# xjtu-omics/SVision

Measured on AMD Instinct MI355X. Metric: candidate SV sites/sec (encode+CNN), higher is better.
Workload: dtype f32

## Files before the change

### include/svx_experimental.h

```cpp
#ifndef SVX_EXPERIMENTAL_H
#define SVX_EXPERIMENTAL_H
#include "svx.h"
#ifdef __cplusplus
extern "C" {
#endif

size_t svx_cigar_scan_flat_ws_bytes(uint64_t n_words_max);
int svx_cigar_scan_flat(const uint32_t* d_cigar, const uint64_t* d_cig_off, const int32_t* d_ref_start, uint32_t n_aln,
                        uint64_t n_words_max, int32_t min_sv, SvxGap* d_gaps, uint64_t gaps_cap, uint32_t* d_gap_off,
                        int32_t* d_stats, void* d_ws, uint64_t ws_bytes, void* stream);

int            svx_bgzf_inflate(const uint8_t* d_comp, const uint64_t* d_src_off, const uint32_t* d_src_len,
                                const uint64_t* d_dst_off, uint32_t n_blocks, uint8_t* d_out, uint32_t* d_status, void* stream);
int            svx_bgzf_inflate_lds(const uint8_t* d_comp, const uint64_t* d_src_off, const uint32_t* d_src_len,
                                    const uint64_t* d_dst_off, uint32_t n_blocks, uint8_t* d_out, uint32_t* d_status, void* stream);
int            svx_bgzf_inflate_private(const uint8_t* d_comp, const uint64_t* d_src_off, const uint32_t* d_src_len,
                                        const uint64_t* d_dst_off, uint32_t n_blocks, uint8_t* d_out, uint32_t* d_status, void* stream);
int            svx_bgzf_inflate_wave(const uint8_t* d_comp, const uint64_t* d_src_off, const uint32_t* d_src_len,
                                     const uint64_t* d_dst_off, uint32_t n_blocks, uint8_t* d_out, uint32_t* d_status, void* stream);

int            svx_bgzf_inflate_fast_lz(const uint8_t* d_comp, const uint64_t* d_src_off, const uint32_t* d_src_len,
                                        const uint64_t* d_dst_off, uint32_t n_blocks, uint64_t inflated_bytes, uint8_t* d_out,
                                        uint32_t* d_status, void* d_ws, uint64_t ws_bytes, int lz_kernel, void* stream_tokens,
                                        void* stream_lz);

#ifdef __cplusplus
}
#endif
#endif
```

### svision_amd/_lib.py

```python
import ctypes
import os

_HERE = os.path.dirname(os.path.abspath(__file__))
LIB_PATH = os.path.join(_HERE, "libsvx.so")

SVX_OK = 0
SVX_EINVAL = -1
SVX_ECAPACITY = -2
SVX_ELAUNCH = -3
LAYOUT_NHWC = 0
LAYOUT_NCHW = 1
IMG = 227
GAP_INS = 1
GAP_DEL = 2

_vp, _u32, _i32, _u64, _sz = ctypes.c_void_p, ctypes.c_uint32, ctypes.c_int32, ctypes.c_uint64, ctypes.c_size_t
SYMBOLS = {
    "svx_version": (ctypes.c_int, []),
    "svx_strerror": (ctypes.c_char_p, [ctypes.c_int]),
    "svx_crc32c": (_u32, [_vp, _sz]),
    "svx_cigar_scan_ws_bytes": (_sz, [_u32, _u64]),
    "svx_cigar_scan": (ctypes.c_int, [_vp, _vp, _vp, _u32, _u64, _i32, _vp, _u64, _vp, _vp, _vp, _u64, _u32, _vp]),
    "svx_rasterize": (ctypes.c_int, [_vp, _u32, _vp, ctypes.c_int, ctypes.POINTER(ctypes.c_float), _vp]),
    "svx_encode_conv1": (ctypes.c_int, [_vp, _u32, _vp, _vp, _vp, ctypes.c_int, _u32, ctypes.c_float, ctypes.c_float,
# ... 54 lines not shown
    "svx_record_retag_measure": (ctypes.c_int, [_vp, _vp, _u32, _vp, _vp, _i32, _vp, _vp, _vp]),
    "svx_record_retag_write": (ctypes.c_int, [_vp, _vp, _u32, _vp, _vp, _i32, _vp, _vp, _vp, _vp]),
    "svx_record_tags_measure": (ctypes.c_int, [_vp, _vp, _u32, _vp, _vp, _vp, _vp]),
    "svx_record_tags_write": (ctypes.c_int, [_vp, _vp, _u32, _vp, _vp, _vp, _vp, _vp]),
    "svx_bgzf_deflate": (ctypes.c_int, [_vp, _vp, _u32, _vp, _vp, _vp, _vp]),
    "svx_bgzf_deflate_dyn_ws_bytes": (_sz, [_u32]),
    "svx_bgzf_deflate_dyn": (ctypes.c_int, [_vp, _vp, _u32, _vp, _vp, _vp, _vp, _u64, _vp]),
    "svx_bgzf_pack": (ctypes.c_int, [_vp, _vp, _u32, _vp, _vp, _u64, _vp]),
    "svx_sam_lines_ws_bytes": (_sz, [_u64]),
    "svx_sam_lines": (ctypes.c_int, [_vp, _u64, _vp, _u64, _vp, _vp, _u64, _vp]),
    "svx_sam_measure": (ctypes.c_int, [_vp, _vp, _u32] + [_vp] * 4 + [_u32] + [_vp] * 5 + [_vp]),
    "svx_sam_encode": (ctypes.c_int, [_vp, _vp, _u32] + [_vp] * 4 + [_u32, _vp, _vp, ctypes.c_int64, _vp, _vp, _vp]),
    "svx_sam_pack_count": (ctypes.c_int, [_vp, _vp, _u32] + [_vp] * 4 + [_u32, ctypes.c_int] + [_vp] * 3 + [_vp]),
    "svx_sam_pack_extract": (ctypes.c_int, [_vp, _vp, _u32] + [_vp] * 4 + [_u32] + [_vp] * 12 + [_vp]),
    "svx_read_range": (ctypes.c_int, [ctypes.c_char_p, _u64, _u64, _vp, ctypes.c_int]),
    "svx_bgzf_index": (ctypes.c_int64, [_vp, _u64, _u64, _u64, _vp, _vp, _vp, _vp, _vp]),
    "svx_name_ids": (ctypes.c_int64, [_vp, _vp, _u64, _vp, _vp, _vp]),
    "svx_stage_open": (_vp, [ctypes.c_char_p, ctypes.c_int, _vp, ctypes.c_int, _vp, ctypes.c_int, _u64, ctypes.c_int, _vp]),
    "svx_stage_group": (ctypes.c_int64, [_vp, _vp, _u64, _vp, _vp, _vp, _u64]),
    "svx_stage_tables": (ctypes.c_int, [_vp, _vp, _vp, _vp, _vp, _u64]),
    "svx_stage_close": (None, [_vp]),
    "svx_bam_stream_open": (_vp, [ctypes.c_char_p, ctypes.c_int, ctypes.c_int, _vp, ctypes.c_int]),
    "svx_bam_stream_next": (_vp, [_vp, _vp]),
    "svx_bam_stream_close": (None, [_vp]),
}
EXPERIMENTAL = {
    "svx_cigar_scan_flat_ws_bytes": (_sz, [_u64]),
    "svx_cigar_scan_flat": (ctypes.c_int, [_vp, _vp, _vp, _u32, _u64, _i32, _vp, _u64, _vp, _vp, _vp, _u64, _vp]),
    "svx_bgzf_inflate": (ctypes.c_int, [_vp, _vp, _vp, _vp, _u32, _vp, _vp, _vp]),
    "svx_bgzf_inflate_wave": (ctypes.c_int, [_vp, _vp, _vp, _vp, _u32, _vp, _vp, _vp]),
    "svx_bgzf_inflate_lds": (ctypes.c_int, [_vp, _vp, _vp, _vp, _u32, _vp, _vp, _vp]),
    "svx_bgzf_inflate_private": (ctypes.c_int, [_vp, _vp, _vp, _vp, _u32, _vp, _vp, _vp]),
    "svx_bgzf_inflate_fast_lz": (ctypes.c_int, [_vp, _vp, _vp, _vp, _u32, _u64, _vp, _vp, _vp, _u64, ctypes.c_int, _vp, _vp]),
}


class SvxError(RuntimeError):
    pass


class SvxMissing(SvxError):
    """libsvx.so has not been built (as opposed to: built, but wrong)."""


_lib = None


ABI_VERSION = 420


def load():
    global _lib
    if _lib is None:
        if not os.path.exists(LIB_PATH):
            raise SvxMissing(
                f"{LIB_PATH} is missing: build it with `python -c 'import __graft_entry__ as g; g.build()'` "
                "or `make -C svision_amd/csrc` (hipcc --offload-arch=gfx950). There is no CPU fallback.")
        lib = ctypes.CDLL(LIB_PATH)
        for name, (res, args) in list(SYMBOLS.items()) + list(EXPERIMENTAL.items()):
            fn = getattr(lib, name)
            fn.restype = res
            fn.argtypes = args
        if lib.svx_version() != ABI_VERSION:
            raise SvxError(f"{LIB_PATH} reports ABI {lib.svx_version()}, this package binds {ABI_VERSION}: rebuild it (make -C svision_amd/csrc)")
        _lib = lib
    return _lib
# ... 7 lines not shown
```

### svision_amd/csrc/svx_dedup.hip

```cpp
#include "svx_raster_common.hpp"

namespace {

constexpr int KEY_BLOCK = 256, COMPACT_BLOCK = 1024, WAVE = 64;

__device__ inline bool key_eq(const uint4& a, const uint4& b) { return a.x == b.x && a.y == b.y && a.z == b.z && a.w == b.w; }

__global__ __launch_bounds__(KEY_BLOCK)
void first_kernel(const int32_t* __restrict__ records, uint32_t n, uint32_t* __restrict__ first, uint4* __restrict__ keys)
{
    __shared__ uint4 tile[KEY_BLOCK];
    const uint32_t i = blockIdx.x * KEY_BLOCK + threadIdx.x;
    const uint4 mine = i < n ? svx_raster::image_key(records + (size_t)i * 12) : uint4{0, 0, 0, 0};
    if (keys && i < n) keys[i] = mine;
    uint32_t f = i;
    for (uint32_t t = 0; t <= blockIdx.x; ++t) {
        const uint32_t j0 = t * KEY_BLOCK;
        __syncthreads();
        if (t == blockIdx.x) tile[threadIdx.x] = mine;
        else tile[threadIdx.x] = svx_raster::image_key(records + (size_t)(j0 + threadIdx.x) * 12);
        __syncthreads();
        if (f == i) {
            const uint32_t hi = min((uint32_t)KEY_BLOCK, i - j0);
            for (uint32_t j = 0; j < hi; ++j)
                if (key_eq(tile[j], mine)) { f = j0 + j; break; }
        }
    }
    if (i < n) first[i] = f;
}

__global__ __launch_bounds__(COMPACT_BLOCK)
void compact_kernel(const int32_t* __restrict__ records, uint32_t n, uint32_t* __restrict__ inv, uint32_t* __restrict__ row,
                    int32_t* __restrict__ unique, uint32_t* __restrict__ live)
{
    __shared__ uint32_t wave_sum[COMPACT_BLOCK / WAVE];
    __shared__ uint32_t s_base;
    const int t = threadIdx.x, lane = t & (WAVE - 1), wv = t / WAVE;
    const uint32_t block = blockDim.x;
    if (t == 0) s_base = 0;
    __syncthreads();
    for (uint32_t c0 = 0; c0 < n; c0 += block) {
        const uint32_t i = c0 + t;
        const bool is_first = i < n && inv[i] == i;
        const unsigned long long ball = __ballot(is_first);
        const uint32_t below = __popcll(ball & ((1ull << lane) - 1ull));
        if (lane == 0) wave_sum[wv] = __popcll(ball);
        __syncthreads();
        uint32_t before = s_base;
        for (int w = 0; w < wv; ++w) before += wave_sum[w];
        if (is_first) {
            const uint32_t c = before + below;
            row[i] = c;
#pragma unroll
            for (int e = 0; e < 12; ++e) unique[(size_t)c * 12 + e] = records[(size_t)i * 12 + e];
        }
        __syncthreads();
        if (t == 0) { uint32_t s = s_base; for (uint32_t w = 0; w < block / WAVE; ++w) s += wave_sum[w]; s_base = s; }
        __syncthreads();
    }
    const uint32_t n_live = s_base;
    for (uint32_t e = n_live * 12 + t; e < n * 12; e += block) unique[e] = records[e % 12];
    for (uint32_t i = t; i < n; i += block) inv[i] = row[inv[i]];
    if (t == 0) *live = n_live;
}

__global__ __launch_bounds__(COMPACT_BLOCK)
void dedup_small_kernel(const int32_t* __restrict__ records, uint32_t n, uint32_t* __restrict__ inv, int32_t* __restrict__ unique,
                        uint32_t* __restrict__ live, uint4* __restrict__ keys)
{
    constexpr uint32_t SCAN = 8;
    __shared__ uint4 tile[COMPACT_BLOCK];
    __shared__ uint32_t row[COMPACT_BLOCK];
    __shared__ uint32_t wave_sum[COMPACT_BLOCK / WAVE];
    const uint32_t i = threadIdx.x, lane = i & (WAVE - 1), wv = i / WAVE, block = blockDim.x;
    const uint4 mine = i < n ? svx_raster::image_key(records + (size_t)i * 12) : uint4{0, 0, 0, 0};
    if (keys && i < n) keys[i] = mine;
    tile[i] = mine;
    __syncthreads();
    uint32_t f = i;
    if (i < n)
        for (uint32_t j0 = 0; j0 < i && f == i; j0 += SCAN) {
            uint32_t hit = 0;
#pragma unroll
            for (uint32_t u = 0; u < SCAN; ++u)
                if (key_eq(tile[j0 + u], mine) && j0 + u < i) hit |= 1u << u;
            if (hit) f = j0 + __ffs(hit) - 1;
        }
    const bool is_first = i < n && f == i;
    const unsigned long long ball = __ballot(is_first);
    const uint32_t below = __popcll(ball & ((1ull << lane) - 1ull));
    if (lane == 0) wave_sum[wv] = __popcll(ball);
    __syncthreads();
    uint32_t before = 0, n_live = 0;
    for (uint32_t w = 0; w < block / WAVE; ++w) { if (w == wv) before = n_live; n_live += wave_sum[w]; }
    if (is_first) {
        const uint32_t c = before + below;
        row[i] = c;
#pragma unroll
        for (int e = 0; e < 12; ++e) unique[(size_t)c * 12 + e] = records[(size_t)i * 12 + e];
    }
    __syncthreads();
    if (i < n) inv[i] = row[f];
    for (uint32_t e = n_live * 12 + i; e < n * 12; e += block) unique[e] = records[e % 12];
    if (i == 0) *live = n_live;
}

__global__ __launch_bounds__(256)
void gather_rows_kernel(const float* __restrict__ src, const uint32_t* __restrict__ inv, float* __restrict__ dst, uint32_t n, uint32_t width)
{
    const uint32_t e = blockIdx.x * 256 + threadIdx.x;
    if (e >= n * width) return;
    const uint32_t i = e / width, c = e - i * width;
    dst[e] = src[(size_t)inv[i] * width + c];
}

}

extern "C" int svx_image_dedup(const int32_t* d_records, uint32_t n, int32_t* d_unique, uint32_t* d_inv, uint32_t* d_live,
                               uint32_t* d_keys, uint32_t* d_ws, void* stream)
{
    if (!d_live) return SVX_EINVAL;
    hipStream_t st = static_cast<hipStream_t>(stream);
    if (n == 0) return hipMemsetAsync(d_live, 0, sizeof(uint32_t), st) == hipSuccess ? SVX_OK : SVX_ELAUNCH;
    if (!d_records || !d_unique || !d_inv || !d_ws || n > (1u << 26)) return SVX_EINVAL;
    if (reinterpret_cast<uintptr_t>(d_keys) & 15u) return SVX_EINVAL;
    const uint32_t block = n >= COMPACT_BLOCK ? COMPACT_BLOCK : (n + WAVE - 1) / WAVE * WAVE;
    if (n <= COMPACT_BLOCK) {
        hipLaunchKernelGGL(dedup_small_kernel, dim3(1), dim3(block), 0, st, d_records, n, d_inv, d_unique, d_live, reinterpret_cast<uint4*>(d_keys));
        return hipGetLastError() == hipSuccess ? SVX_OK : SVX_ELAUNCH;
    }
    hipLaunchKernelGGL(first_kernel, dim3((n + KEY_BLOCK - 1) / KEY_BLOCK), dim3(KEY_BLOCK), 0, st, d_records, n, d_inv,
                       reinterpret_cast<uint4*>(d_keys));
    hipLaunchKernelGGL(compact_kernel, dim3(1), dim3(block), 0, st, d_records, n, d_inv, d_ws, d_unique, d_live);
    return hipGetLastError() == hipSuccess ? SVX_OK : SVX_ELAUNCH;
}

extern "C" int svx_gather_rows(const float* d_src, const uint32_t* d_inv, float* d_dst, uint32_t n, uint32_t width, void* stream)
{
    if (n == 0 || width == 0) return SVX_OK;
    if (!d_src || !d_inv || !d_dst || (uint64_t)n * width > 0xffffffffull) return SVX_EINVAL;
    const uint32_t total = n * width;
    hipLaunchKernelGGL(gather_rows_kernel, dim3((total + 255) / 256), dim3(256), 0, static_cast<hipStream_t>(stream), d_src, d_inv, d_dst, n, width);
    return hipGetLastError() == hipSuccess ? SVX_OK : SVX_ELAUNCH;
}
```

### svision_amd/csrc/svx_inflate2.hip

```cpp
#include <hip/hip_runtime.h>
#include <stdint.h>
#include <stdlib.h>
#include "../../include/svx.h"
#include "svx_lz_core.hpp"
#include "svx_lz_table_core.hpp"
#include "svx_wave_scan.hpp"

#ifndef SVX_TOK_DBG
#define SVX_TOK_DBG 0
#endif

namespace {

constexpr int LANES = 64;
#ifndef SVX_TOK_LB
#define SVX_TOK_LB 9
#define SVX_TOK_DB 7
#endif
#ifndef SVX_TOK_WAVES
#define SVX_TOK_WAVES 4
#endif
constexpr int LB = SVX_TOK_LB, DB = SVX_TOK_DB;
constexpr int LIT_CAP = (1 << LB) + (LB >= 9 ? 340 : 512), DIST_CAP = (1 << DB) + 528;
#ifndef SVX_TOK_SEG
#define SVX_TOK_SEG 512
#endif
constexpr int SEG_BITS = SVX_TOK_SEG;
constexpr int CHUNK_WORDS = LANES * SEG_BITS / 32 + 8;
enum { K_BAD = 0, K_LIT = 1, K_LEN = 2, K_EOB = 3, K_SUB = 4 };
enum { INF_OK = 0, INF_BAD_TYPE = 1, INF_BAD_STORED = 2, INF_BAD_TABLE = 3, INF_BAD_CODE = 4, INF_OUT_OVERRUN = 5, INF_IN_OVERRUN = 6, INF_SHORT = 7,
       INF_BAD_DIST = 8, INF_TOKENS_OVERFLOW = 10 };

__constant__ uint16_t LEN_BASE[29] = {3, 4, 5, 6, 7, 8, 9, 10, 11, 13, 15, 17, 19, 23, 27, 31, 35, 43, 51, 59, 67, 83, 99, 115, 131, 163, 195, 227, 258};
__constant__ uint8_t LEN_EXTRA[29] = {0, 0, 0, 0, 0, 0, 0, 0, 1, 1, 1, 1, 2, 2, 2, 2, 3, 3, 3, 3, 4, 4, 4, 4, 5, 5, 5, 5, 0};
__constant__ uint16_t DIST_BASE[30] = {1, 2, 3, 4, 5, 7, 9, 13, 17, 25, 33, 49, 65, 97, 129, 193, 257, 385, 513, 769, 1025, 1537, 2049, 3073, 4097, 6145, 8193, 12289, 16385, 24577};
__constant__ uint8_t DIST_EXTRA[30] = {0, 0, 0, 0, 1, 1, 2, 2, 3, 3, 4, 4, 5, 5, 6, 6, 7, 7, 8, 8, 9, 9, 10, 10, 11, 11, 12, 12, 13, 13};
__constant__ uint8_t CLEN_ORDER[19] = {16, 17, 18, 0, 8, 7, 9, 6, 10, 5, 11, 4, 12, 3, 13, 2, 14, 1, 15};

struct LitPayload {
    __device__ __forceinline__ uint32_t operator()(int s) const
    {
        if (s < 256) return (uint32_t)K_LIT << 4 | (uint32_t)s << 8;
        if (s == 256) return (uint32_t)K_EOB << 4;
        if (s - 257 >= 29) return (uint32_t)K_BAD << 4;
        return (uint32_t)K_LEN << 4 | (uint32_t)LEN_BASE[s - 257] << 8 | (uint32_t)LEN_EXTRA[s - 257] << 17;
    }
};
struct DistPayload {
    __device__ __forceinline__ uint32_t operator()(int s) const
    {
        return s >= 30 ? (uint32_t)K_BAD << 4 : ((uint32_t)K_LEN << 4 | (uint32_t)DIST_BASE[s] << 8 | (uint32_t)DIST_EXTRA[s] << 23);
    }
};
struct ClenPayload { __device__ __forceinline__ uint32_t operator()(int s) const { return (uint32_t)K_LIT << 4 | (uint32_t)s << 8; } };

struct Lds {
    uint32_t lit[LIT_CAP];
    uint32_t dist[DIST_CAP];
    uint32_t chunk[CHUNK_WORDS];
    __device__ __forceinline__ uint8_t* lens() { return reinterpret_cast<uint8_t*>(chunk) + 1024; }
    __device__ __forceinline__ uint8_t* cl() { return reinterpret_cast<uint8_t*>(chunk) + 1344; }
    __device__ __forceinline__ uint16_t* code() { return reinterpret_cast<uint16_t*>(chunk) + 704; }
};
static_assert(sizeof(Lds) <= 10240 && LANES * SEG_BITS / 8 >= 2048, "sixteen waves per CU; the builder's scratch fits the chunk buffer");

__device__ __forceinline__ int uni(int v) { return __builtin_amdgcn_readfirstlane(v); }
__device__ __forceinline__ void lds_fence() { __builtin_amdgcn_s_waitcnt(0xc07f); __builtin_amdgcn_wave_barrier(); }

struct HeadReader {
    const uint32_t* words;
    uint32_t cur, nxt;
    uint64_t chunk_next, word_end;
    int k;
    uint64_t buf;
    int cnt;
    uint32_t fed;
    __device__ __forceinline__ uint32_t fetch(uint64_t first) { const uint64_t i = first + threadIdx.x; return i < word_end ? words[i] : 0u; }
    __device__ __forceinline__ void refill()
    {
        if (cnt <= 32) {
            const uint32_t v = (uint32_t)__builtin_amdgcn_readlane((int)cur, k);
            if (++k == 64) { cur = nxt; nxt = fetch(chunk_next); chunk_next += 64; k = 0; }
            buf |= (uint64_t)v << cnt;
            cnt += 32;
        }
    }
    __device__ __forceinline__ void seek(const uint8_t* base, uint32_t bytes, uint32_t bit)
    {
        const uintptr_t a = reinterpret_cast<uintptr_t>(base) + (bit >> 3);
        words = reinterpret_cast<const uint32_t*>(a & ~(uintptr_t)3);
        word_end = ((reinterpret_cast<uintptr_t>(base) + bytes + 3) >> 2) - (reinterpret_cast<uintptr_t>(words) >> 2) + 1;
        cur = fetch(0); nxt = fetch(64); chunk_next = 128;
        k = 0; buf = 0; cnt = 0;
        refill();
        const int skip = (int)(a & 3) * 8 + (int)(bit & 7);
        buf >>= skip; cnt -= skip;
        fed = 0;
    }
    __device__ __forceinline__ uint32_t bits(int n)
    {
        refill();
        const uint32_t v = (uint32_t)buf & ((1u << n) - 1u);
        buf >>= n; cnt -= n; fed += (uint32_t)n;
        return v;
    }
};

template <class Payload>
__device__ int build_tables(const uint8_t* lens, int n, int root, uint32_t* tab, int cap, uint16_t* code_of, uint8_t* tmp, Payload payload)
{
    const int lane = threadIdx.x;
    const unsigned long long lt = (1ull << lane) - 1ull;
    int count[16];
#pragma unroll
    for (int l = 0; l < 16; ++l) count[l] = 0;
    for (int s0 = 0; s0 < n; s0 += LANES) {
        const int l = s0 + lane < n ? (int)lens[s0 + lane] : 0;
#pragma unroll
        for (int q = 1; q < 16; ++q) count[q] += (int)__popcll(__ballot(l == q));
    }
    int next[16], left = 1, code = 0;
    next[0] = 0;
#pragma unroll
    for (int l = 1; l <= 15; ++l) {
        left = (left << 1) - count[l];
        code = (code + (l > 1 ? count[l - 1] : 0)) << 1;
        next[l] = code;
    }
    if (left < 0) return 0;
    for (int s0 = 0; s0 < n; s0 += LANES) {
        const int l = s0 + lane < n ? (int)lens[s0 + lane] : 0;
        int mine = 0;
#pragma unroll
        for (int q = 1; q < 16; ++q) {
            const unsigned long long m = __ballot(l == q);
            if (l == q) mine = next[q] + (int)__popcll(m & lt);
            next[q] += (int)__popcll(m);
        }
        if (s0 + lane < n) code_of[s0 + lane] = (uint16_t)mine;
    }
    const int nroot = 1 << root;
    for (int i = lane; i < nroot; i += LANES) { tab[i] = 0; tmp[i] = 0; }
    lds_fence();
    for (int s0 = 0; s0 < n; s0 += LANES) {
// ... 73 lines not shown
    Tok k{(e >> 4) & 15u, used, (e >> 8) & 255u, 0u, 0u};
    if (k.kind != K_LEN) return k;
    const uint32_t xb = (e >> 17) & 7u;
    k.len = ((e >> 8) & 511u) + ((b.lo >> used) & ((1u << xb) - 1u));
    used += xb;
    const uint32_t db32 = __builtin_amdgcn_alignbit(b.hi, b.lo, used);
    uint32_t d = t.dist[db32 & ((1u << DB) - 1u)];
    uint32_t dused;
    if (((d >> 4) & 15u) == K_SUB) {
        d = t.dist[((d >> 8) & 0xfffu) + ((db32 >> DB) & ((1u << ((d >> 20) & 15u)) - 1u))];
        dused = DB + (d & 15u);
    } else dused = d & 15u;
    if (((d >> 4) & 15u) != K_LEN) { k.kind = K_BAD; k.used = used + dused; return k; }
    const uint32_t nb = (d >> 23) & 15u;
    k.dist = ((d >> 8) & 0x7fffu) + ((db32 >> dused) & ((1u << nb) - 1u));
    k.used = used + dused + nb;
    return k;
}

using svx_wave::wave_incl_scan;

__device__ __forceinline__ uint32_t wave_excl_sum(uint32_t v, uint32_t* total)
{
    const uint32_t inc = wave_incl_scan(v);
    *total = (uint32_t)__builtin_amdgcn_readlane((int)inc, LANES - 1);
    return inc - v;
}

__host__ __device__ inline uint64_t stream_base(const uint64_t* dst_off, uint32_t b) { return svx_lzt::slot_base(dst_off, b); }

__device__ __forceinline__ void put32(uint8_t* p, uint32_t v) { __builtin_memcpy(p, &v, 4); }

template <bool SPLIT>
__global__ __launch_bounds__(LANES) __attribute__((amdgpu_waves_per_eu(SVX_TOK_WAVES, 8)))
void bgzf_tokens_kernel(const uint8_t* __restrict__ comp, const uint64_t* __restrict__ src_off, const uint32_t* __restrict__ src_len,
                        const uint64_t* __restrict__ dst_off, uint32_t n_blocks, uint8_t* __restrict__ streams, uint2* __restrict__ stream_cnt,
                        uint32_t* __restrict__ status)
{
    __shared__ Lds t;
    const uint32_t b = blockIdx.x;
    const int lane = threadIdx.x;
    const uint8_t* src = comp + src_off[b];
    const uint32_t nbytes = src_len[b], nbits = nbytes * 8u;
    const uint32_t isize = (uint32_t)(dst_off[b + 1] - dst_off[b]);
    uint8_t* stream = streams + stream_base(dst_off, b);
    const uint32_t cap = (uint32_t)(stream_base(dst_off, b + 1) - stream_base(dst_off, b));
    const uint32_t pad = SPLIT ? (uint32_t)(-(intptr_t)reinterpret_cast<uintptr_t>(stream)) & 3u : 0u;
    uint8_t* const hdr0 = stream + pad;
    uint8_t* const lit_end = stream + cap;
    uint32_t P = 0, W = 0, Q = pad;
    uint32_t H = 0, Lc = 0;
    int err = INF_OK;
    bool last = false;
    HeadReader hr;
    while (!last && err == INF_OK) {
        hr.seek(src, nbytes, P);
        last = hr.bits(1) != 0;
        const uint32_t type = hr.bits(2);
        if (type == 0) {
            hr.bits((int)((P + hr.fed) & 7u ? 8u - ((P + hr.fed) & 7u) : 0u));
            const uint32_t len = hr.bits(16), nlen = hr.bits(16);
            P += hr.fed;
            if ((len ^ nlen) != 0xffffu) { err = INF_BAD_STORED; break; }
            if (W + len > isize) { err = INF_OUT_OVERRUN; break; }
            if (P + 8u * len > nbits) { err = INF_IN_OVERRUN; break; }
            const uint32_t nseq = (len + 254u) / 255u;
            if (Q + len + 4u * nseq > cap) { err = INF_TOKENS_OVERFLOW; break; }
            const uint8_t* from = src + (P >> 3);
            for (uint32_t s = lane; s < nseq; s += LANES) {
                const uint32_t n = min(255u, len - 255u * s);
                if (SPLIT) {
                    put32(hdr0 + 4u * (H + s), n);
                    uint8_t* q = lit_end - 1 - (Lc + 255u * s);
                    for (uint32_t i = 0; i < n; ++i) q[-(int)i] = from[255u * s + i];
// ... 128 lines not shown
                while (__any(run)) {
                    const bool go = run && p < f;
                    Tok k{K_EOB, 0u, 0u, 0u, 0u};
                    if (go) k = token(t, p - bit0);
                    p += k.used;
                    const bool isl = go && k.kind == K_LIT, ism = go && k.kind == K_LEN;
                    const bool full = isl && nl == 255u;
                    if (full) put32(hdr, 255u);
                    hdr += full ? (SPLIT ? 4 : 259) : 0;
                    nl = full ? 0u : nl;
                    if (SPLIT) { lp -= isl ? 1 : 0; if (isl) *lp = (uint8_t)k.val; }
                    else if (isl) hdr[4 + nl] = (uint8_t)k.val;
                    if (ism) put32(hdr, nl | k.len << 8 | (k.dist - 1u) << 17);
                    const bool far = ism && k.dist > w;
                    bad_dist = bad_dist || far;
                    hdr += ism ? (SPLIT ? 4 : 4 + nl) : 0;
                    nl = ism ? 0u : nl + (isl ? 1u : 0u);
                    w += ism ? k.len : isl ? 1u : 0u;
                    run = (isl || ism) && !far;
                }
                if (valid && nl) put32(hdr, nl);
                if (__any(bad_dist)) { err = INF_BAD_DIST; break; }
            }
            W += tot_o; Q += tot_e;
            if (SPLIT) { Lc += tot_e - 4u * tot_h; H += tot_h; }
            if (first < LANES) { eob = true; P = (uint32_t)__shfl((int)f, first, LANES); }
            else P = (uint32_t)__shfl((int)f, LANES - 1, LANES);
        }
    }
    if (err == INF_OK && W != isize) err = INF_SHORT;
    if (lane == 0) { status[b] = (uint32_t)err; stream_cnt[b] = SPLIT ? make_uint2(H, Lc) : make_uint2(Q, 0u); }
}

constexpr int LZ_LANES = 64, RING_STRIDE = svx_lz::RING + 16;

__global__ __launch_bounds__(LZ_LANES)
void bgzf_lz_kernel(const uint8_t* __restrict__ streams, const uint2* __restrict__ stream_cnt, const uint64_t* __restrict__ dst_off,
                    uint32_t n_blocks, uint8_t* out, uint32_t* __restrict__ status)
{
    extern __shared__ __attribute__((aligned(16))) uint8_t rings[];
    const uint32_t b = blockIdx.x * LZ_LANES + threadIdx.x;
    if (b >= n_blocks) return;
    if (status[b] != 0) return;
    const int err = svx_lz::decode_block(streams + stream_base(dst_off, b), stream_cnt[b].x, out, dst_off[b], dst_off[b + 1],
                                         rings + threadIdx.x * RING_STRIDE);
    if (err != svx_lz::LZ_OK) status[b] = (uint32_t)err;
}


constexpr int WAVE_LZ_BELOW = 12000;
constexpr uint32_t WRING = 32768, WMASK = WRING - 1, WSTAGE = 4096, WFLUSH = 4096;

__global__ __launch_bounds__(LANES)
void bgzf_lz_wave_kernel(const uint8_t* __restrict__ streams, const uint2* __restrict__ stream_cnt, const uint64_t* __restrict__ dst_off,
                         uint32_t n_blocks, uint8_t* out, uint32_t* __restrict__ status)
{
    extern __shared__ __attribute__((aligned(16))) uint8_t wlds[];
    uint8_t* const ring = wlds;
    uint8_t* const stage = wlds + WRING;
    const uint32_t b = blockIdx.x;
    const uint32_t lane = threadIdx.x;
    if (status[b] != 0) return;
    const uint64_t lo = dst_off[b], hi = dst_off[b + 1];
    if (hi == lo) return;
    const uint32_t nseq = stream_cnt[b].x, nlit = stream_cnt[b].y;
    const uint8_t* slot = streams + stream_base(dst_off, b);
// ... 99 lines not shown
                if (__any(act && i8 < nl)) {
                    if (act && i8 < nl) ring[(w32 + i8) & WMASK] = stage[((L + m.z + 16u - r + i8) ^ 15u) & (WSTAGE - 1)];
                }
                if (act && rd) ring[(w32 + nl + i8) & WMASK] = ring[(base32 + (uint32_t)srel) & WMASK];
                k0 += n_ok;
            } else {
                careful((uint32_t)__builtin_amdgcn_readfirstlane((int32_t)m.x), W + (uint32_t)step0, L + (uint32_t)__builtin_amdgcn_readfirstlane((int32_t)m.z));
                if (err != svx_lz::LZ_OK) break;
                k0 += 1;
            }
        }
        W += T; L += Lt;
        if ((uint32_t)((uint32_t)W - (uint32_t)flushed) >= WFLUSH + 16u) flush_to(W & ~15ull);
    }
    if (err == svx_lz::LZ_OK && W != hi) err = svx_lz::LZ_SHORT;
    if (err == svx_lz::LZ_OK) flush_to(hi);
    else if (lane == 0) status[b] = (uint32_t)err;
}

}

extern "C" size_t svx_bgzf_inflate_fast_ws_bytes(uint64_t inflated_bytes, uint32_t n_blocks)
{
    return (size_t)((((size_t)8 * n_blocks + 255) & ~(size_t)255) + inflated_bytes + (inflated_bytes >> 1) + 1024ull * n_blocks + 64);
}

extern "C" __attribute__((visibility("hidden"))) int svx_bgzf_inflate_wave_only(const uint8_t* d_comp, const uint64_t* d_src_off, const uint32_t* d_src_len, const uint64_t* d_dst_off,
                                          uint32_t n_blocks, uint8_t* d_out, uint32_t* d_status, uint32_t only, void* stream);

extern "C" __attribute__((visibility("hidden"))) int svx_bgzf_lz_table_available(void);
extern "C" __attribute__((visibility("hidden"))) int svx_bgzf_lz_table(const uint8_t* streams, const void* stream_cnt, const uint64_t* d_dst_off, uint32_t n_blocks,
                                                                        uint8_t* d_out, uint32_t* d_status, uint32_t handover, void* stream);

extern "C" int svx_bgzf_inflate_fast_lz(const uint8_t* d_comp, const uint64_t* d_src_off, const uint32_t* d_src_len, const uint64_t* d_dst_off,
                                        uint32_t n_blocks, uint64_t inflated_bytes, uint8_t* d_out, uint32_t* d_status, void* d_ws, uint64_t ws_bytes,
                                        int lz_kernel, void* stream_tokens, void* stream_lz)
{
    if (n_blocks == 0) return SVX_OK;
    if (!d_comp || !d_src_off || !d_src_len || !d_dst_off || !d_out || !d_status || !d_ws) return SVX_EINVAL;
    if (reinterpret_cast<uintptr_t>(d_ws) & 15u) return SVX_EINVAL;
    if (ws_bytes < svx_bgzf_inflate_fast_ws_bytes(inflated_bytes, n_blocks)) return SVX_EINVAL;
    hipStream_t sa = static_cast<hipStream_t>(stream_tokens), sb = static_cast<hipStream_t>(stream_lz);
    uint2* stream_cnt = static_cast<uint2*>(d_ws);
    uint8_t* streams = static_cast<uint8_t*>(d_ws) + (((size_t)8 * n_blocks + 255) & ~(size_t)255);
    static const uint32_t below = getenv("SVX_WAVE_LZ_BELOW") ? (uint32_t)atoi(getenv("SVX_WAVE_LZ_BELOW")) : (uint32_t)WAVE_LZ_BELOW;
    if (lz_kernel < 0 || lz_kernel > 3) return SVX_EINVAL;
    if (lz_kernel == 3 && !svx_bgzf_lz_table_available()) return SVX_EINVAL;
    const bool table_lz = lz_kernel ? lz_kernel == 3 : svx_bgzf_lz_table_available() != 0;
    const bool wave_lz = table_lz || (lz_kernel ? lz_kernel == 2 : n_blocks < below);
    const char* only = getenv("SVX_INFLATE2_ONLY");
    if (!only && getenv("SVX_INFLATE2_ONLY_A")) only = "A";
    if (!only || only[0] != 'B') {
        if (sa != sb) {
            hipEvent_t ready;
            if (hipEventCreateWithFlags(&ready, hipEventDisableTiming) != hipSuccess) return SVX_ELAUNCH;
            (void)hipEventRecord(ready, sb);
            (void)hipStreamWaitEvent(sa, ready, 0);
            (void)hipEventDestroy(ready);
        }
        static const unsigned tok_lds = getenv("SVX_TOK_LDS") ? (unsigned)atoi(getenv("SVX_TOK_LDS")) : 0u;
        if (wave_lz) hipLaunchKernelGGL(bgzf_tokens_kernel<true>, dim3(n_blocks), dim3(LANES), tok_lds, sa, d_comp, d_src_off, d_src_len, d_dst_off, n_blocks, streams, stream_cnt, d_status);
        else hipLaunchKernelGGL(bgzf_tokens_kernel<false>, dim3(n_blocks), dim3(LANES), tok_lds, sa, d_comp, d_src_off, d_src_len, d_dst_off, n_blocks, streams, stream_cnt, d_status);
        if (sa != sb) {
            hipEvent_t done;
            if (hipEventCreateWithFlags(&done, hipEventDisableTiming) != hipSuccess) return SVX_ELAUNCH;
            (void)hipEventRecord(done, sa);
            (void)hipStreamWaitEvent(sb, done, 0);
            (void)hipEventDestroy(done);
        }
    }
    if (only && only[0] == 'A') return SVX_OK;
    if (table_lz) { if (svx_bgzf_lz_table(streams, stream_cnt, d_dst_off, n_blocks, d_out, d_status, INF_TOKENS_OVERFLOW, sb) != SVX_OK) return SVX_ELAUNCH; }
    else if (wave_lz) hipLaunchKernelGGL(bgzf_lz_wave_kernel, dim3(n_blocks), dim3(LANES), WRING + WSTAGE + 1024, sb, streams, stream_cnt, d_dst_off, n_blocks, d_out, d_status);
    else hipLaunchKernelGGL(bgzf_lz_kernel, dim3((n_blocks + LZ_LANES - 1) / LZ_LANES), dim3(LZ_LANES), LZ_LANES * RING_STRIDE, sb, streams, stream_cnt, d_dst_off, n_blocks, d_out, d_status);
    if (hipGetLastError() != hipSuccess) return SVX_ELAUNCH;
    return svx_bgzf_inflate_wave_only(d_comp, d_src_off, d_src_len, d_dst_off, n_blocks, d_out, d_status, INF_TOKENS_OVERFLOW, stream_lz);
}

extern "C" int svx_bgzf_inflate_fast_on(const uint8_t* d_comp, const uint64_t* d_src_off, const uint32_t* d_src_len, const uint64_t* d_dst_off,
                                        uint32_t n_blocks, uint64_t inflated_bytes, uint8_t* d_out, uint32_t* d_status, void* d_ws, uint64_t ws_bytes,
                                        void* stream_tokens, void* stream_lz)
{
    return svx_bgzf_inflate_fast_lz(d_comp, d_src_off, d_src_len, d_dst_off, n_blocks, inflated_bytes, d_out, d_status, d_ws, ws_bytes, 0, stream_tokens, stream_lz);
}

extern "C" int svx_bgzf_inflate_fast(const uint8_t* d_comp, const uint64_t* d_src_off, const uint32_t* d_src_len, const uint64_t* d_dst_off,
                                     uint32_t n_blocks, uint64_t inflated_bytes, uint8_t* d_out, uint32_t* d_status, void* d_ws, uint64_t ws_bytes,
                                     void* stream)
{
    return svx_bgzf_inflate_fast_on(d_comp, d_src_off, d_src_len, d_dst_off, n_blocks, inflated_bytes, d_out, d_status, d_ws, ws_bytes, stream, stream);
}
```

### svision_amd/kernels.py

```python
import collections
import ctypes

import numpy as np
import torch

from . import _lib

GAP_DTYPE = np.dtype([("aln", "<u4"), ("op", "<u4"), ("read_pos", "<i4"),
                      ("ref_pos", "<i4"), ("len", "<i4"), ("kind", "<u4")])
MEAN = (104.0, 117.0, 124.0)


def to_c8(x):
    n, c, h, w = x.shape
    if c % 8:
        raise _lib.SvxError("the C8 layout needs a channel count that is a multiple of 8")
    return x.reshape(n, c // 8, 8, h, w).permute(0, 1, 3, 4, 2).contiguous()


def from_c8(x):
    n, o, h, w, e = x.shape
    return x.permute(0, 1, 4, 2, 3).reshape(n, o * e, h, w).contiguous()


# ... 582 lines not shown


def inflate_variant_for(n_blocks):
    import os
    variant = os.environ.get("SVX_INFLATE_VARIANT", "fast")
    if variant == "auto":
        return "wave" if n_blocks < WAVE_KERNEL_BELOW else "lane"
    return variant


def inflate_workspace(lib, variant, inflated_bytes, n_blocks, device):
    if not variant.startswith("fast"):
        return None
    return torch.empty(int(lib.svx_bgzf_inflate_fast_ws_bytes(int(inflated_bytes), int(n_blocks))), dtype=torch.uint8, device=device)


def launch_inflate(lib, variant, comp_ptr, src_ptr, len_ptr, dst_ptr, n_blocks, out_ptr, status_ptr, inflated_bytes, device, ws=None, tokens_stream=None):
    st = _stream_ptr(device)
    lz = None
    if variant in ("fast-lane", "fast-wave", "fast-table"):
        lz, variant = variant[5:], "fast"
    if variant == "fast":
        d_ws = ws if ws is not None else inflate_workspace(lib, variant, inflated_bytes, n_blocks, device)
        ws_bytes = int(d_ws.numel())
        rc = _launch_fast(lib, comp_ptr, src_ptr, len_ptr, dst_ptr, n_blocks, inflated_bytes, out_ptr, status_ptr, d_ws, ws_bytes, tokens_stream, st, lz)
        _lib.check(rc, "svx_bgzf_inflate (%s)" % variant)
        return
    fn = {"lds": lib.svx_bgzf_inflate_lds, "private": lib.svx_bgzf_inflate_private, "wave": lib.svx_bgzf_inflate_wave,
          "lane": lib.svx_bgzf_inflate}[variant]
    rc = fn(comp_ptr, src_ptr, len_ptr, dst_ptr, n_blocks, out_ptr, status_ptr, st)
    _lib.check(rc, "svx_bgzf_inflate (%s)" % variant)


def _launch_fast(lib, comp_ptr, src_ptr, len_ptr, dst_ptr, n_blocks, inflated_bytes, out_ptr, status_ptr, d_ws, ws_bytes, tokens_stream, st, lz=None):
    if lz is not None:
        tok = ctypes.c_void_p(tokens_stream.cuda_stream) if tokens_stream is not None else st
        return lib.svx_bgzf_inflate_fast_lz(comp_ptr, src_ptr, len_ptr, dst_ptr, n_blocks, int(inflated_bytes), out_ptr, status_ptr, d_ws.data_ptr(), ws_bytes,
                                            {"lane": 1, "wave": 2, "table": 3}[lz], tok, st)
    if tokens_stream is not None:
        return lib.svx_bgzf_inflate_fast_on(comp_ptr, src_ptr, len_ptr, dst_ptr, n_blocks, int(inflated_bytes), out_ptr, status_ptr, d_ws.data_ptr(), ws_bytes,
                                            ctypes.c_void_p(tokens_stream.cuda_stream), st)
    return lib.svx_bgzf_inflate_fast(comp_ptr, src_ptr, len_ptr, dst_ptr, n_blocks, int(inflated_bytes), out_ptr, status_ptr, d_ws.data_ptr(), ws_bytes, st)


INFLATE_BAD_CRC = 9


def bgzf_crc_wanted():
    import os
    return os.environ.get("SVX_BGZF_CRC", "1") != "0"


def bgzf_inflate(d_comp, src_off, src_len, isize, wave=None, crc=None):
    lib = _lib.load()
    _require_cuda(d_comp, "d_comp")
    if d_comp.dtype != torch.uint8:
        raise _lib.SvxError("d_comp must be a uint8 tensor")
    n = int(len(src_off))
    dev = d_comp.device
    dst = np.zeros(n + 1, np.uint64)
    dst[1:] = np.cumsum(np.asarray(isize, np.uint64))
    total = int(dst[-1])
    d_out = torch.empty(max(total, 4), dtype=torch.uint8, device=dev)
    d_status = torch.zeros(max(n, 1), dtype=torch.int32, device=dev)
    if n:
        d_src = torch.from_numpy(np.ascontiguousarray(src_off, np.uint64).view(np.int64)).to(dev)
        d_len = torch.from_numpy(np.ascontiguousarray(src_len, np.uint32).view(np.int32)).to(dev)
# ... 429 lines not shown
```

Baseline: 8062.

## Add persistent-grid option for BGZF token kernel and move LDS to dynamic

Turns the token-decoding kernel into a grid-stride loop so it can run as a persistent grid sized by CU count times a residency factor. Moves its LDS struct and the small dedup kernel's shared arrays to dynamic shared memory. Raises the default minimum waves-per-EU hint for the token kernel from 4 to 5. The persistent mode is opt-in through an environment variable, so by default the grid still equals the block count; the waves-per-EU change alters register allocation by default and may cause spills.

```diff
diff --git a/include/svx_experimental.h b/include/svx_experimental.h
--- a/include/svx_experimental.h
+++ b/include/svx_experimental.h
@@ -24,6 +24,11 @@
                                         uint32_t* d_status, void* d_ws, uint64_t ws_bytes, int lz_kernel, void* stream_tokens,
                                         void* stream_lz);
 
+int            svx_bgzf_inflate_fast_resident(const uint8_t* d_comp, const uint64_t* d_src_off, const uint32_t* d_src_len,
+                                              const uint64_t* d_dst_off, uint32_t n_blocks, uint64_t inflated_bytes, uint8_t* d_out,
+                                              uint32_t* d_status, void* d_ws, uint64_t ws_bytes, int lz_kernel, uint32_t tok_residency,
+                                              uint32_t tok_grid, void* stream_tokens, void* stream_lz);
+
 #ifdef __cplusplus
 }
 #endif
diff --git a/svision_amd/_lib.py b/svision_amd/_lib.py
--- a/svision_amd/_lib.py
+++ b/svision_amd/_lib.py
@@ -110,6 +110,7 @@
     "svx_bgzf_inflate_lds": (ctypes.c_int, [_vp, _vp, _vp, _vp, _u32, _vp, _vp, _vp]),
     "svx_bgzf_inflate_private": (ctypes.c_int, [_vp, _vp, _vp, _vp, _u32, _vp, _vp, _vp]),
     "svx_bgzf_inflate_fast_lz": (ctypes.c_int, [_vp, _vp, _vp, _vp, _u32, _u64, _vp, _vp, _vp, _u64, ctypes.c_int, _vp, _vp]),
+    "svx_bgzf_inflate_fast_resident": (ctypes.c_int, [_vp, _vp, _vp, _vp, _u32, _u64, _vp, _vp, _vp, _u64, ctypes.c_int, _u32, _u32, _vp, _vp]),
 }
 
 
diff --git a/svision_amd/csrc/svx_dedup.hip b/svision_amd/csrc/svx_dedup.hip
--- a/svision_amd/csrc/svx_dedup.hip
+++ b/svision_amd/csrc/svx_dedup.hip
@@ -3,6 +3,8 @@
 namespace {
 
 constexpr int KEY_BLOCK = 256, COMPACT_BLOCK = 1024, WAVE = 64;
+
+constexpr uint32_t dedup_small_lds(uint32_t block) { return block * (uint32_t)(sizeof(uint4) + sizeof(uint32_t)) + block / WAVE * (uint32_t)sizeof(uint32_t); }
 
 __device__ inline bool key_eq(const uint4& a, const uint4& b) { return a.x == b.x && a.y == b.y && a.z == b.z && a.w == b.w; }
 
@@ -69,10 +71,11 @@
                         uint32_t* __restrict__ live, uint4* __restrict__ keys)
 {
     constexpr uint32_t SCAN = 8;
-    __shared__ uint4 tile[COMPACT_BLOCK];
-    __shared__ uint32_t row[COMPACT_BLOCK];
-    __shared__ uint32_t wave_sum[COMPACT_BLOCK / WAVE];
+    extern __shared__ __attribute__((aligned(16))) uint8_t dedup_lds[];
     const uint32_t i = threadIdx.x, lane = i & (WAVE - 1), wv = i / WAVE, block = blockDim.x;
+    uint4* const tile = reinterpret_cast<uint4*>(dedup_lds);
+    uint32_t* const row = reinterpret_cast<uint32_t*>(dedup_lds + (size_t)block * sizeof(uint4));
+    uint32_t* const wave_sum = row + block;
     const uint4 mine = i < n ? svx_raster::image_key(records + (size_t)i * 12) : uint4{0, 0, 0, 0};
     if (keys && i < n) keys[i] = mine;
     tile[i] = mine;
@@ -126,7 +129,7 @@
     if (reinterpret_cast<uintptr_t>(d_keys) & 15u) return SVX_EINVAL;
     const uint32_t block = n >= COMPACT_BLOCK ? COMPACT_BLOCK : (n + WAVE - 1) / WAVE * WAVE;
     if (n <= COMPACT_BLOCK) {
-        hipLaunchKernelGGL(dedup_small_kernel, dim3(1), dim3(block), 0, st, d_records, n, d_inv, d_unique, d_live, reinterpret_cast<uint4*>(d_keys));
+        hipLaunchKernelGGL(dedup_small_kernel, dim3(1), dim3(block), dedup_small_lds(block), st, d_records, n, d_inv, d_unique, d_live, reinterpret_cast<uint4*>(d_keys));
         return hipGetLastError() == hipSuccess ? SVX_OK : SVX_ELAUNCH;
     }
     hipLaunchKernelGGL(first_kernel, dim3((n + KEY_BLOCK - 1) / KEY_BLOCK), dim3(KEY_BLOCK), 0, st, d_records, n, d_inv,
diff --git a/svision_amd/csrc/svx_inflate2.hip b/svision_amd/csrc/svx_inflate2.hip
--- a/svision_amd/csrc/svx_inflate2.hip
+++ b/svision_amd/csrc/svx_inflate2.hip
@@ -1,6 +1,8 @@
 #include <hip/hip_runtime.h>
 #include <stdint.h>
 #include <stdlib.h>
+#include <algorithm>
+#include <atomic>
 #include "../../include/svx.h"
 #include "svx_lz_core.hpp"
 #include "svx_lz_table_core.hpp"
@@ -18,7 +20,7 @@
 #define SVX_TOK_DB 7
 #endif
 #ifndef SVX_TOK_WAVES
-#define SVX_TOK_WAVES 4
+#define SVX_TOK_WAVES 5
 #endif
 constexpr int LB = SVX_TOK_LB, DB = SVX_TOK_DB;
 constexpr int LIT_CAP = (1 << LB) + (LB >= 9 ? 340 : 512), DIST_CAP = (1 << DB) + 528;
@@ -64,6 +66,7 @@
 };
 static_assert(sizeof(Lds) <= 10240 && LANES * SEG_BITS / 8 >= 2048, "sixteen waves per CU; the builder's scratch fits the chunk buffer");
 
+__device__ __forceinline__ int lane_id() { int l = threadIdx.x; asm volatile("" : "+v"(l)); return l; }
 __device__ __forceinline__ int uni(int v) { return __builtin_amdgcn_readfirstlane(v); }
 __device__ __forceinline__ void lds_fence() { __builtin_amdgcn_s_waitcnt(0xc07f); __builtin_amdgcn_wave_barrier(); }
 
@@ -75,7 +78,7 @@
     uint64_t buf;
     int cnt;
     uint32_t fed;
-    __device__ __forceinline__ uint32_t fetch(uint64_t first) { const uint64_t i = first + threadIdx.x; return i < word_end ? words[i] : 0u; }
+    __device__ __forceinline__ uint32_t fetch(uint64_t first) { const uint64_t i = first + lane_id(); return i < word_end ? words[i] : 0u; }
     __device__ __forceinline__ void refill()
     {
         if (cnt <= 32) {
@@ -109,7 +112,7 @@
 template <class Payload>
 __device__ int build_tables(const uint8_t* lens, int n, int root, uint32_t* tab, int cap, uint16_t* code_of, uint8_t* tmp, Payload payload)
 {
-    const int lane = threadIdx.x;
+    const int lane = lane_id();
     const unsigned long long lt = (1ull << lane) - 1ull;
     int count[16];
 #pragma unroll
@@ -249,14 +252,11 @@
 __device__ __forceinline__ void put32(uint8_t* p, uint32_t v) { __builtin_memcpy(p, &v, 4); }
 
 template <bool SPLIT>
-__global__ __launch_bounds__(LANES) __attribute__((amdgpu_waves_per_eu(SVX_TOK_WAVES, 8)))
-void bgzf_tokens_kernel(const uint8_t* __restrict__ comp, const uint64_t* __restrict__ src_off, const uint32_t* __restrict__ src_len,
-                        const uint64_t* __restrict__ dst_off, uint32_t n_blocks, uint8_t* __restrict__ streams, uint2* __restrict__ stream_cnt,
-                        uint32_t* __restrict__ status)
-{
-    __shared__ Lds t;
-    const uint32_t b = blockIdx.x;
-    const int lane = threadIdx.x;
+__device__ __forceinline__ void tokens_block(Lds& t, const uint32_t b, const uint8_t* __restrict__ comp, const uint64_t* __restrict__ src_off,
+                                             const uint32_t* __restrict__ src_len, const uint64_t* __restrict__ dst_off, uint8_t* __restrict__ streams,
+                                             uint2* __restrict__ stream_cnt, uint32_t* __restrict__ status)
+{
+    const int lane = lane_id();
     const uint8_t* src = comp + src_off[b];
     const uint32_t nbytes = src_len[b], nbits = nbytes * 8u;
     const uint32_t isize = (uint32_t)(dst_off[b + 1] - dst_off[b]);
@@ -451,6 +451,18 @@
     if (lane == 0) { status[b] = (uint32_t)err; stream_cnt[b] = SPLIT ? make_uint2(H, Lc) : make_uint2(Q, 0u); }
 }
 
+template <bool SPLIT>
+__global__ __launch_bounds__(LANES) __attribute__((amdgpu_waves_per_eu(SVX_TOK_WAVES, 8)))
+void bgzf_tokens_kernel(const uint8_t* __restrict__ comp, const uint64_t* __restrict__ src_off, const uint32_t* __restrict__ src_len,
+                        const uint64_t* __restrict__ dst_off, uint32_t n_blocks, uint8_t* __restrict__ streams, uint2* __restrict__ stream_cnt,
+                        uint32_t* __restrict__ status)
+{
+    extern __shared__ __attribute__((aligned(16))) uint8_t tok_lds_raw[];
+    Lds& t = *reinterpret_cast<Lds*>(tok_lds_raw);
+    for (uint32_t b = blockIdx.x; b < n_blocks; b += gridDim.x)
+        tokens_block<SPLIT>(t, b, comp, src_off, src_len, dst_off, streams, stream_cnt, status);
+}
+
 constexpr int LZ_LANES = 64, RING_STRIDE = svx_lz::RING + 16;
 
 __global__ __launch_bounds__(LZ_LANES)
@@ -616,9 +628,26 @@
 extern "C" __attribute__((visibility("hidden"))) int svx_bgzf_lz_table(const uint8_t* streams, const void* stream_cnt, const uint64_t* d_dst_off, uint32_t n_blocks,
                                                                         uint8_t* d_out, uint32_t* d_status, uint32_t handover, void* stream);
 
-extern "C" int svx_bgzf_inflate_fast_lz(const uint8_t* d_comp, const uint64_t* d_src_off, const uint32_t* d_src_len, const uint64_t* d_dst_off,
-                                        uint32_t n_blocks, uint64_t inflated_bytes, uint8_t* d_out, uint32_t* d_status, void* d_ws, uint64_t ws_bytes,
-                                        int lz_kernel, void* stream_tokens, void* stream_lz)
+constexpr uint32_t TOK_RESIDENCY_DEFAULT = 0;
+static uint32_t tokens_grid(uint32_t n_blocks, uint32_t tok_residency, uint32_t tok_grid)
+{
+    if (tok_grid) return tok_grid;
+    if (!tok_residency) return n_blocks;
+    static std::atomic<int> cus_of[64];
+    int dev = 0, cus = 0;
+    if (hipGetDevice(&dev) != hipSuccess) return 0;
+    const bool known = dev >= 0 && dev < 64;
+    if (known) cus = cus_of[dev].load(std::memory_order_relaxed);
+    if (cus <= 0) {
+        if (hipDeviceGetAttribute(&cus, hipDeviceAttributeMultiprocessorCount, dev) != hipSuccess || cus <= 0) return 0;
+        if (known) cus_of[dev].store(cus, std::memory_order_relaxed);
+    }
+    return (uint32_t)std::min<uint64_t>(n_blocks, (uint64_t)cus * tok_residency);
+}
+
+extern "C" int svx_bgzf_inflate_fast_resident(const uint8_t* d_comp, const uint64_t* d_src_off, const uint32_t* d_src_len, const uint64_t* d_dst_off,
+                                              uint32_t n_blocks, uint64_t inflated_bytes, uint8_t* d_out, uint32_t* d_status, void* d_ws, uint64_t ws_bytes,
+                                              int lz_kernel, uint32_t tok_residency, uint32_t tok_grid, void* stream_tokens, void* stream_lz)
 {
     if (n_blocks == 0) return SVX_OK;
     if (!d_comp || !d_src_off || !d_src_len || !d_dst_off || !d_out || !d_status || !d_ws) return SVX_EINVAL;
@@ -629,6 +658,7 @@
     uint8_t* streams = static_cast<uint8_t*>(d_ws) + (((size_t)8 * n_blocks + 255) & ~(size_t)255);
     static const uint32_t below = getenv("SVX_WAVE_LZ_BELOW") ? (uint32_t)atoi(getenv("SVX_WAVE_LZ_BELOW")) : (uint32_t)WAVE_LZ_BELOW;
     if (lz_kernel < 0 || lz_kernel > 3) return SVX_EINVAL;
+    if (tok_residency > 64u || tok_grid > (1u << 20)) return SVX_EINVAL;
     if (lz_kernel == 3 && !svx_bgzf_lz_table_available()) return SVX_EINVAL;
     const bool table_lz = lz_kernel ? lz_kernel == 3 : svx_bgzf_lz_table_available() != 0;
     const bool wave_lz = table_lz || (lz_kernel ? lz_kernel == 2 : n_blocks < below);
@@ -642,9 +672,11 @@
             (void)hipStreamWaitEvent(sa, ready, 0);
             (void)hipEventDestroy(ready);
         }
-        static const unsigned tok_lds = getenv("SVX_TOK_LDS") ? (unsigned)atoi(getenv("SVX_TOK_LDS")) : 0u;
-        if (wave_lz) hipLaunchKernelGGL(bgzf_tokens_kernel<true>, dim3(n_blocks), dim3(LANES), tok_lds, sa, d_comp, d_src_off, d_src_len, d_dst_off, n_blocks, streams, stream_cnt, d_status);
-        else hipLaunchKernelGGL(bgzf_tokens_kernel<false>, dim3(n_blocks), dim3(LANES), tok_lds, sa, d_comp, d_src_off, d_src_len, d_dst_off, n_blocks, streams, stream_cnt, d_status);
+        static const unsigned tok_lds = (unsigned)sizeof(Lds) + (getenv("SVX_TOK_LDS") ? (unsigned)atoi(getenv("SVX_TOK_LDS")) : 0u);
+        const uint32_t grid = tokens_grid(n_blocks, tok_residency, tok_grid);
+        if (!grid) return SVX_ELAUNCH;
+        if (wave_lz) hipLaunchKernelGGL(bgzf_tokens_kernel<true>, dim3(grid), dim3(LANES), tok_lds, sa, d_comp, d_src_off, d_src_len, d_dst_off, n_blocks, streams, stream_cnt, d_status);
+        else hipLaunchKernelGGL(bgzf_tokens_kernel<false>, dim3(grid), dim3(LANES), tok_lds, sa, d_comp, d_src_off, d_src_len, d_dst_off, n_blocks, streams, stream_cnt, d_status);
         if (sa != sb) {
             hipEvent_t done;
             if (hipEventCreateWithFlags(&done, hipEventDisableTiming) != hipSuccess) return SVX_ELAUNCH;
@@ -661,6 +693,14 @@
     return svx_bgzf_inflate_wave_only(d_comp, d_src_off, d_src_len, d_dst_off, n_blocks, d_out, d_status, INF_TOKENS_OVERFLOW, stream_lz);
 }
 
+extern "C" int svx_bgzf_inflate_fast_lz(const uint8_t* d_comp, const uint64_t* d_src_off, const uint32_t* d_src_len, const uint64_t* d_dst_off,
+                                        uint32_t n_blocks, uint64_t inflated_bytes, uint8_t* d_out, uint32_t* d_status, void* d_ws, uint64_t ws_bytes,
+                                        int lz_kernel, void* stream_tokens, void* stream_lz)
+{
+    return svx_bgzf_inflate_fast_resident(d_comp, d_src_off, d_src_len, d_dst_off, n_blocks, inflated_bytes, d_out, d_status, d_ws, ws_bytes, lz_kernel,
+                                          TOK_RESIDENCY_DEFAULT, 0, stream_tokens, stream_lz);
+}
+
 extern "C" int svx_bgzf_inflate_fast_on(const uint8_t* d_comp, const uint64_t* d_src_off, const uint32_t* d_src_len, const uint64_t* d_dst_off,
                                         uint32_t n_blocks, uint64_t inflated_bytes, uint8_t* d_out, uint32_t* d_status, void* d_ws, uint64_t ws_bytes,
                                         void* stream_tokens, void* stream_lz)
diff --git a/svision_amd/kernels.py b/svision_amd/kernels.py
--- a/svision_amd/kernels.py
+++ b/svision_amd/kernels.py
@@ -638,7 +638,18 @@
     _lib.check(rc, "svx_bgzf_inflate (%s)" % variant)
 
 
+def tokens_residency():
+    import os
+    v = os.environ.get("SVX_TOK_RESIDENCY", "")
+    return int(v) if v else None
+
+
 def _launch_fast(lib, comp_ptr, src_ptr, len_ptr, dst_ptr, n_blocks, inflated_bytes, out_ptr, status_ptr, d_ws, ws_bytes, tokens_stream, st, lz=None):
+    residency = tokens_residency()
+    if residency is not None:
+        tok = ctypes.c_void_p(tokens_stream.cuda_stream) if tokens_stream is not None else st
+        return lib.svx_bgzf_inflate_fast_resident(comp_ptr, src_ptr, len_ptr, dst_ptr, n_blocks, int(inflated_bytes), out_ptr, status_ptr, d_ws.data_ptr(), ws_bytes,
+                                                  {None: 0, "lane": 1, "wave": 2, "table": 3}[lz], residency, 0, tok, st)
     if lz is not None:
         tok = ctypes.c_void_p(tokens_stream.cuda_stream) if tokens_stream is not None else st
         return lib.svx_bgzf_inflate_fast_lz(comp_ptr, src_ptr, len_ptr, dst_ptr, n_blocks, int(inflated_bytes), out_ptr, status_ptr, d_ws.data_ptr(), ws_bytes,
```

Result: faster. 8294 (median of 4 runs) (+2.9%).
